# i2Nav-WHU/IC-GVINS

Hardware: AMD Instinct MI355X
Metric: frames/s at 1280x720, 300 feats, 10-KF window; residual/Jacobian eval/s (higher is better)
Workload: dtype u8/int64 front-end (f32/f64 solves), f64 factors

## Files before the change

### ic-gvins_amd/csrc/image.hip

```cpp
#include <algorithm>

#include "icg_internal.h"

#define PRE_MAX_JOBS 64
struct pre_jobs {
    const uint8_t *src[PRE_MAX_JOBS];
    int32_t slot[PRE_MAX_JOBS];
    int stride;
    const int32_t *slot_ind;
};
__device__ __forceinline__ int pre_job_slot(const pre_jobs &j, int b) { return j.slot_ind ? j.slot_ind[b] : j.slot[b]; }

__global__ void k_bgr2gray(const uint8_t *bgr, int w, int h, int sstride, size_t sbatch, uint8_t *gray, int gstride,
                           size_t gbatch) {
    int x = blockIdx.x * blockDim.x + threadIdx.x;
    int y = blockIdx.y;
    int b = blockIdx.z;
    if (x >= w) return;
    const uint8_t *p = bgr + (size_t) b * sbatch + (size_t) y * sstride + 3 * x;
    gray[(size_t) b * gbatch + (size_t) y * gstride + x] =
        (uint8_t) ((p[0] * 1868 + p[1] * 9617 + p[2] * 4899 + 8192) >> 14);
}

__global__ void k_hist256(pre_jobs jobs, int w, int h, unsigned int *hist ) {
    __shared__ unsigned int sh[256];
    int b = blockIdx.y;
    sh[threadIdx.x] = 0;
    __syncthreads();
    const uint8_t *src = jobs.src[b];
    const int stride   = jobs.stride;
    int total          = src ? w * h : 0;
    for (int i = blockIdx.x * blockDim.x + threadIdx.x; i < total; i += gridDim.x * blockDim.x) {
        int y = i / w, x = i - y * w;
        atomicAdd(&sh[src[(size_t) y * stride + x]], 1u);
    }
    __syncthreads();
    if (sh[threadIdx.x]) atomicAdd(&hist[(size_t) b * 256 + threadIdx.x], sh[threadIdx.x]);
}

struct clahe_geom {
    int w, h, tw, th, clip;
    float lut_scale, inv_tw, inv_th;
};

__device__ __forceinline__ int wave_sum_i32(int v) {
    v += __builtin_amdgcn_update_dpp(0, v, 0xB1, 0xF, 0xF, false);
    v += __builtin_amdgcn_update_dpp(0, v, 0x4E, 0xF, 0xF, false);
    v += __builtin_amdgcn_update_dpp(0, v, 0x141, 0xF, 0xF, false);
    v += __builtin_amdgcn_update_dpp(0, v, 0x140, 0xF, 0xF, false);
    v += __builtin_amdgcn_update_dpp(0, v, 0x142, 0xA, 0xF, false);
    v += __builtin_amdgcn_update_dpp(0, v, 0x143, 0xC, 0xF, false);
    return __builtin_amdgcn_readlane(v, 63);
}
__device__ __forceinline__ int wave_scan_i32(int v) {
    v += __builtin_amdgcn_update_dpp(0, v, 0x111, 0xF, 0xF, true);
    v += __builtin_amdgcn_update_dpp(0, v, 0x112, 0xF, 0xF, true);
    v += __builtin_amdgcn_update_dpp(0, v, 0x114, 0xF, 0xF, true);
    v += __builtin_amdgcn_update_dpp(0, v, 0x118, 0xF, 0xF, true);
    v += __builtin_amdgcn_update_dpp(0, v, 0x142, 0xA, 0xF, false);
    v += __builtin_amdgcn_update_dpp(0, v, 0x143, 0xC, 0xF, false);
    return v;
}

__global__ __launch_bounds__(64) void k_clahe_lut(pre_jobs jobs, clahe_geom g, uint8_t *lut , int n_items) {
    __shared__ __attribute__((aligned(16))) unsigned int hist[256];
    const int lane = threadIdx.x;
    const int item = icg_xcd_chunked(blockIdx.x, n_items);
    if (item >= n_items) return;
    const int b    = item / (ICG_CLAHE_TILES * ICG_CLAHE_TILES);
    const int tile = item - b * (ICG_CLAHE_TILES * ICG_CLAHE_TILES);
    const int ty = tile / ICG_CLAHE_TILES, tx = tile - ty * ICG_CLAHE_TILES;
    const uint8_t *src = jobs.src[b];
    if (!src) return;
    const int stride   = jobs.stride;
    reinterpret_cast<uint4 *>(hist)[lane] = make_uint4(0, 0, 0, 0);
    __syncthreads();

    const int x_begin = tx * g.tw, x_end = x_begin + g.tw, y_begin = ty * g.th;
    const int xa  = x_begin & ~3;
    const int ndw = (((x_end + 3) & ~3) - xa) >> 2;
    const bool pad_small = g.th * ICG_CLAHE_TILES < 2 * g.h - 1;
    auto load_row_dword = [&](int r, int x) -> unsigned int {
        const uint8_t *row = src + (size_t) (pad_small ? icg_reflect1(y_begin + r, g.h) : icg_reflect101(y_begin + r, g.h)) * stride;
        if (x + 3 < g.w) return *reinterpret_cast<const unsigned int *>(row + x);
        unsigned int v = 0;
#pragma unroll
        for (int j = 0; j < 4; j++) v |= (unsigned int) row[icg_reflect101(x + j, g.w)] << (8 * j);
        return v;
    };
    const int nin = ndw - 2;
    const bool fast = nin >= 1 && nin <= 16 && y_begin + g.th <= g.h && xa + 4 * ndw <= g.w;
    if (fast) {
        const int d = lane & 15, q = lane >> 4;
        const bool on = d < nin;
        const uint8_t *p = src + (size_t) (y_begin + q) * stride + (xa + 4 * (on ? d + 1 : 1));
        unsigned char *hb = reinterpret_cast<unsigned char *>(hist);
        const size_t step = 4 * (size_t) stride;
        for (int r = q; r < g.th; r += 16, p += 4 * step) {
            unsigned int v[4];
            bool ok[4];
#pragma unroll
            for (int k = 0; k < 4; k++) {
                ok[k] = on && r + 4 * k < g.th;
                v[k]  = r + 4 * k < g.th ? *reinterpret_cast<const unsigned int *>(p + k * step) : 0u;
            }
#pragma unroll
            for (int k = 0; k < 4; k++) {
                if (ok[k]) {
                    atomicAdd(reinterpret_cast<unsigned int *>(hb + ((v[k] << 2) & 0x3fcu)), 1u);
                    atomicAdd(reinterpret_cast<unsigned int *>(hb + ((v[k] >> 6) & 0x3fcu)), 1u);
                    atomicAdd(reinterpret_cast<unsigned int *>(hb + ((v[k] >> 14) & 0x3fcu)), 1u);
                    atomicAdd(reinterpret_cast<unsigned int *>(hb + ((v[k] >> 22) & 0x3fcu)), 1u);
                }
            }
        }
    } else {
        {
            const int items = g.th * (nin > 0 ? nin : 0);
            const unsigned int magic = nin > 0 ? ((1u << 20) + (unsigned int) nin - 1u) / (unsigned int) nin : 0u;
            constexpr int CH = 9;
            for (int base = 0; base < items; base += 64 * CH) {
                unsigned int v[CH];
                bool ok[CH];
    #pragma unroll
                for (int k = 0; k < CH; k++) {
                    const int i = base + k * 64 + lane;
                    ok[k]       = i < items;
                    v[k]        = 0;
                    if (ok[k]) {
                        const int r = (int) (((unsigned int) i * magic) >> 20), d = 1 + i - r * nin;
                        v[k]        = load_row_dword(r, xa + 4 * d);
                    }
                }
    #pragma unroll
                for (int k = 0; k < CH; k++) {
                    if (ok[k]) {
    #pragma unroll
                        for (int j = 0; j < 4; j++) atomicAdd(&hist[(v[k] >> (8 * j)) & 0xff], 1u);
                    }
                }
            }
        }
    }
    {
        const int nedge = ndw >= 2 ? 2 : 1, items = g.th * nedge;
        for (int i = lane; i < items; i += 64) {
            const int r = nedge == 2 ? (i >> 1) : i, d = (nedge == 2 && (i & 1)) ? ndw - 1 : 0;
            const int x = xa + 4 * d;
            const unsigned int v = load_row_dword(r, x);
#pragma unroll
            for (int j = 0; j < 4; j++) {
                const int xx = x + j;
                if (xx >= x_begin && xx < x_end) atomicAdd(&hist[(v >> (8 * j)) & 0xff], 1u);
            }
        }
    }
    __syncthreads();

    const uint4 h4 = reinterpret_cast<const uint4 *>(hist)[lane];
    int hv[4]      = {(int) h4.x, (int) h4.y, (int) h4.z, (int) h4.w};
    int excess     = 0;
#pragma unroll
    for (int j = 0; j < 4; j++) {
        if (hv[j] > g.clip) {
            excess += hv[j] - g.clip;
            hv[j] = g.clip;
        }
    }
    const int clipped   = wave_sum_i32(excess);
    const int batch_add = clipped / 256;
    const int residual  = clipped - batch_add * 256;
    int step            = residual ? 256 / residual : 1;
    if (step < 1) step = 1;
    int run = 0;
#pragma unroll
    for (int j = 0; j < 4; j++) {
        const int t = 4 * lane + j;
        hv[j] += batch_add;
        if (residual != 0 && (t % step) == 0 && (t / step) < residual) hv[j]++;
        run += hv[j];
        hv[j] = run;
    }
    const int incl = wave_scan_i32(run);
    const int excl = incl - run;
    unsigned int packed = 0;
#pragma unroll
    for (int j = 0; j < 4; j++) {
        const float f = rintf((float) (excl + hv[j]) * g.lut_scale);
        int iv        = (int) f;
        iv            = iv < 0 ? 0 : (iv > 255 ? 255 : iv);
        packed |= (unsigned int) iv << (8 * j);
    }
    reinterpret_cast<unsigned int *>(lut + ((size_t) b * ICG_CLAHE_TILES * ICG_CLAHE_TILES + tile) * 256)[lane] = packed;
}

#define CLAHE_CHUNK 256
#define CLAHE_MAXCOLS 24
#define CLAHE_FCOLS 8

typedef float f32x2 __attribute__((ext_vector_type(2)));

template <bool FLT>
__device__ __forceinline__ void clahe_apply_body(const pre_jobs &jobs, const clahe_geom &g, const uint8_t *lut, uint8_t *frames, size_t slot_bytes,
                                                 int dpitch, unsigned int *slut, int strip, int chunk, int b, int t, int dslot, int p_lo, int npairs,
                                                 int x_begin) {
    const int T = ICG_CLAHE_TILES;
    int ty1 = strip - 1, ty2 = strip;
    if (ty1 < 0) ty1 = 0;
    if (ty2 > T - 1) ty2 = T - 1;
    const unsigned int *blut = reinterpret_cast<const unsigned int *>(lut + (size_t) b * T * T * 256);
    for (int i = t; i < npairs * 64; i += 256) {
        const int p = p_lo + (i >> 6), v4 = i & 63;
        int c1 = p - 1, c2 = p;
        if (c1 < 0) c1 = 0;
        if (c2 > T - 1) c2 = T - 1;
        const unsigned int A = blut[(ty1 * T + c1) * 64 + v4], B = blut[(ty1 * T + c2) * 64 + v4];
        const unsigned int C = blut[(ty2 * T + c1) * 64 + v4], D = blut[(ty2 * T + c2) * 64 + v4];
        if (FLT) {
            float4 *dst = reinterpret_cast<float4 *>(slut) + 4 * i;
#define CL_F(w, k) ((float) (((w) >> (8 * (k))) & 0xffu))
            dst[0] = make_float4(CL_F(A, 0), CL_F(B, 0), CL_F(C, 0), CL_F(D, 0));
            dst[1] = make_float4(CL_F(A, 1), CL_F(B, 1), CL_F(C, 1), CL_F(D, 1));
            dst[2] = make_float4(CL_F(A, 2), CL_F(B, 2), CL_F(C, 2), CL_F(D, 2));
            dst[3] = make_float4(CL_F(A, 3), CL_F(B, 3), CL_F(C, 3), CL_F(D, 3));
#undef CL_F
        } else {
            const unsigned int ab01 = __builtin_amdgcn_perm(B, A, 0x05010400u), ab23 = __builtin_amdgcn_perm(B, A, 0x07030602u);
            const unsigned int cd01 = __builtin_amdgcn_perm(D, C, 0x05010400u), cd23 = __builtin_amdgcn_perm(D, C, 0x07030602u);
            uint4 e;
            e.x = __builtin_amdgcn_perm(cd01, ab01, 0x05040100u);
            e.y = __builtin_amdgcn_perm(cd01, ab01, 0x07060302u);
            e.z = __builtin_amdgcn_perm(cd23, ab23, 0x05040100u);
            e.w = __builtin_amdgcn_perm(cd23, ab23, 0x07060302u);
            reinterpret_cast<uint4 *>(slut)[i] = e;
        }
    }
    __syncthreads();

    const int wave = t >> 6, lane = t & 63;
    const int x0 = x_begin + lane * 4;
    int pofs[4];
    float xa[4], xa1[4];
#pragma unroll
    for (int k = 0; k < 4; k++) {
        const int x     = x0 + k;
        const float txf = x * g.inv_tw - 0.5f;
        const int tx1   = (int) floorf(txf);
        xa[k]           = txf - tx1;
        xa1[k]          = 1.0f - xa[k];
        int p           = tx1 + 1 - p_lo;
        p               = p < 0 ? 0 : (p > npairs - 1 ? npairs - 1 : p);
        pofs[k]         = p << 8;
    }
    if (x0 >= g.w) return;

    int y_lo = (strip - 1) * g.th + g.th / 2 - 2;
    int y_hi = strip * g.th + g.th / 2 + 3;
    if (y_lo < 0) y_lo = 0;
    if (y_hi > g.h) y_hi = g.h;
    const uint8_t *src = jobs.src[b];
    const int stride   = jobs.stride;
    uint8_t *dst       = frames + (size_t) dslot * slot_bytes;
    if (FLT) {
        const float4 *sf = reinterpret_cast<const float4 *>(slut);
        for (int y = y_lo + wave; y < y_hi; y += 4) {
            const float tyf = y * g.inv_th - 0.5f;
            const int tyr   = (int) floorf(tyf);
            if (tyr != strip - 1) continue;
            const float ya = tyf - tyr, ya1 = 1.0f - ya;
            const unsigned int pin = *reinterpret_cast<const unsigned int *>(src + (size_t) y * stride + x0);
            const float4 e0 = sf[pofs[0] + (pin & 0xff)], e1 = sf[pofs[1] + ((pin >> 8) & 0xff)];
            const float4 e2 = sf[pofs[2] + ((pin >> 16) & 0xff)], e3 = sf[pofs[3] + (pin >> 24)];
            const float r0 = (e0.x * xa1[0] + e0.y * xa[0]) * ya1 + (e0.z * xa1[0] + e0.w * xa[0]) * ya;
            const float r1 = (e1.x * xa1[1] + e1.y * xa[1]) * ya1 + (e1.z * xa1[1] + e1.w * xa[1]) * ya;
            const float r2 = (e2.x * xa1[2] + e2.y * xa[2]) * ya1 + (e2.z * xa1[2] + e2.w * xa[2]) * ya;
            const float r3 = (e3.x * xa1[3] + e3.y * xa[3]) * ya1 + (e3.z * xa1[3] + e3.w * xa[3]) * ya;
            const unsigned int m0 = __float_as_uint(r0 + 12582912.f), m1 = __float_as_uint(r1 + 12582912.f);
            const unsigned int m2 = __float_as_uint(r2 + 12582912.f), m3 = __float_as_uint(r3 + 12582912.f);
            const unsigned int lo = __builtin_amdgcn_perm(m1, m0, 0x0c0c0400u), hi = __builtin_amdgcn_perm(m3, m2, 0x0c0c0400u);
            *reinterpret_cast<unsigned int *>(dst + (size_t) y * dpitch + x0) = __builtin_amdgcn_perm(hi, lo, 0x05040100u);
        }
        return;
    }
    const f32x2 XA01 = {xa[0], xa[1]}, XA23 = {xa[2], xa[3]}, XB01 = {xa1[0], xa1[1]}, XB23 = {xa1[2], xa1[3]};
    for (int y = y_lo + wave; y < y_hi; y += 4) {
        const float tyf = y * g.inv_th - 0.5f;
        const int tyr   = (int) floorf(tyf);
        if (tyr != strip - 1) continue;
        const float ya = tyf - tyr, ya1 = 1.0f - ya;
        const unsigned int pin = *reinterpret_cast<const unsigned int *>(src + (size_t) y * stride + x0);
        const unsigned int e0 = slut[pofs[0] + (pin & 0xff)], e1 = slut[pofs[1] + ((pin >> 8) & 0xff)];
        const unsigned int e2 = slut[pofs[2] + ((pin >> 16) & 0xff)], e3 = slut[pofs[3] + (pin >> 24)];
#define CL_B(e, k) ((float) (((e) >> (8 * (k))) & 0xffu))
        const f32x2 A01 = {CL_B(e0, 0), CL_B(e1, 0)}, B01 = {CL_B(e0, 1), CL_B(e1, 1)};
        const f32x2 C01 = {CL_B(e0, 2), CL_B(e1, 2)}, D01 = {CL_B(e0, 3), CL_B(e1, 3)};
        const f32x2 A23 = {CL_B(e2, 0), CL_B(e3, 0)}, B23 = {CL_B(e2, 1), CL_B(e3, 1)};
        const f32x2 C23 = {CL_B(e2, 2), CL_B(e3, 2)}, D23 = {CL_B(e2, 3), CL_B(e3, 3)};
#undef CL_B
        const f32x2 r01 = (A01 * XB01 + B01 * XA01) * ya1 + (C01 * XB01 + D01 * XA01) * ya;
        const f32x2 r23 = (A23 * XB23 + B23 * XA23) * ya1 + (C23 * XB23 + D23 * XA23) * ya;
        const float res[4] = {r01.x, r01.y, r23.x, r23.y};
        unsigned int pout = 0;
#pragma unroll
        for (int k = 0; k < 4; k++) {
            const int iv = (int) rintf(res[k]);
            pout |= (unsigned int) (iv < 0 ? 0 : (iv > 255 ? 255 : iv)) << (8 * k);
        }
        *reinterpret_cast<unsigned int *>(dst + (size_t) y * dpitch + x0) = pout;
    }
}

__global__ __launch_bounds__(256) void k_clahe_apply(pre_jobs jobs, clahe_geom g, const uint8_t *lut, uint8_t *frames,
                                                     size_t slot_bytes, int dpitch) {
    __shared__ __attribute__((aligned(16))) unsigned int slut[CLAHE_FCOLS * 256 * 4];
    static_assert(CLAHE_FCOLS * 4 >= CLAHE_MAXCOLS, "the byte form must fit the same array");
    const int strip = blockIdx.x;
    const int chunk = blockIdx.y;
    const int b     = blockIdx.z;
    const int t     = threadIdx.x;
    const int dslot = pre_job_slot(jobs, b);
    if (!jobs.src[b] || dslot < 0) return;
    const int x_begin = chunk * CLAHE_CHUNK;
    int x_end         = x_begin + CLAHE_CHUNK;
    if (x_end > g.w) x_end = g.w;
    const int p_lo   = (int) floorf(x_begin * g.inv_tw - 0.5f) + 1;
    const int p_hi   = (int) floorf((x_end - 1) * g.inv_tw - 0.5f) + 1;
    const int npairs = p_hi - p_lo + 1;
    if (npairs <= CLAHE_FCOLS)
        clahe_apply_body<true>(jobs, g, lut, frames, slot_bytes, dpitch, slut, strip, chunk, b, t, dslot, p_lo, npairs, x_begin);
    else
        clahe_apply_body<false>(jobs, g, lut, frames, slot_bytes, dpitch, slut, strip, chunk, b, t, dslot, p_lo, npairs, x_begin);
}

#define PR_STRIP_OUT 128
struct pr_sel {
    unsigned int a, b, t, v;
};
typedef unsigned int pr_u3 __attribute__((ext_vector_type(3)));
__device__ __forceinline__ pr_u3 pr_load(const uint8_t *row, unsigned int wx) {
    typedef pr_u3 __attribute__((aligned(4))) u3a;
    return *reinterpret_cast<const u3a *>(row + wx);
}
template <bool EDGE> __device__ __forceinline__ unsigned int pr_hsum(const pr_u3 E, const pr_sel &S) {
    unsigned int A, B, V4;
    if (EDGE) {
        A  = __builtin_amdgcn_perm(E.y, E.x, S.a);
        B  = __builtin_amdgcn_perm(E.y, E.x, S.b);
        V4 = __builtin_amdgcn_perm(E.z, __builtin_amdgcn_perm(E.y, E.x, S.t), S.v);
    } else {
        A  = __builtin_amdgcn_alignbyte(E.y, E.x, 2);
        B  = E.y;
        V4 = E.z & 0xffu;
    }
    const unsigned int h0 = __builtin_amdgcn_udot4(B, 0x00010000u, __builtin_amdgcn_udot4(A, 0x04060401u, 0u, false), false);
    const unsigned int h1 = __builtin_amdgcn_udot4(B, 0x04060401u, V4, false);
    return h0 | (h1 << 16);
}

template <bool EDGE>
__device__ __forceinline__ void pr_band(const uint8_t *src, int sh, int spitch, uint8_t *dst, int dpitch, int i0, int i1, unsigned int wx,
                                        const pr_sel &S, unsigned int dcol, bool store) {
    auto srow = [&](int r) { return src + (unsigned int) __builtin_amdgcn_readfirstlane(icg_reflect1(r, sh) * spitch); };
    unsigned int hA = pr_hsum<EDGE>(pr_load(srow(2 * i0 - 2), wx), S), hB = pr_hsum<EDGE>(pr_load(srow(2 * i0 - 1), wx), S);
    unsigned int hC = pr_hsum<EDGE>(pr_load(srow(2 * i0), wx), S);
    pr_u3 R1 = pr_load(srow(2 * i0 + 1), wx), R2 = pr_load(srow(2 * i0 + 2), wx);
    for (int i = i0; i < i1; i++) {
        const pr_u3 N1 = pr_load(srow(2 * i + 3), wx), N2 = pr_load(srow(2 * i + 4), wx);
        const unsigned int hD = pr_hsum<EDGE>(R1, S), hE = pr_hsum<EDGE>(R2, S);
        unsigned int v = hA + hE;
        v              = ((hB + hD) << 2) + v;
        v += (hC << 2) + (hC + hC);
        v += 0x00800080u;
        if (store) *reinterpret_cast<unsigned short *>(dst + (size_t) i * dpitch + dcol) = (unsigned short) __builtin_amdgcn_perm(v, v, 0x0c0c0301u);
        hA = hC, hB = hD, hC = hE;
        R1 = N1, R2 = N2;
    }
}

__global__ __launch_bounds__(64) void k_pyrdown_rows(uint8_t *frames, size_t slot_bytes, pre_jobs jobs, unsigned int src_off, int sw, int sh,
                                                     int spitch, unsigned int dst_off, int dw, int dh, int dpitch, int n_strips, int n_bands,
                                                     int band_rows, int n_tasks) {
    const int task = icg_xcd_chunked(blockIdx.x, n_tasks);
    if (task >= n_tasks) return;
    const int per_job = n_strips * n_bands;
    const int job = task / per_job, rem = task - job * per_job;
    const int band = rem / n_strips, strip = rem - band * n_strips;
    const int dslot = __builtin_amdgcn_readfirstlane(pre_job_slot(jobs, job));
    if (dslot < 0) return;
    uint8_t *slot = frames + (size_t) dslot * slot_bytes;
    const int lane = threadIdx.x;
    const int oj   = strip * PR_STRIP_OUT + 2 * lane;
    const int x  = min(2 * oj, (sw - 1) & ~3);
    const int wx = max(x - 4, 0);
    const bool edge = strip == 0 || 2 * (strip + 1) * PR_STRIP_OUT + 4 > sw;
    pr_sel S;
    S.a = S.b = S.t = S.v = 0;
    if (edge) {
        int ix[7];
#pragma unroll
        for (int k = 0; k < 7; k++) ix[k] = min(max(icg_reflect101(x - 2 + k, sw) - wx, 0), 11);
        S.a = (unsigned int) (ix[0] & 7) | ((unsigned int) (ix[1] & 7) << 8) | ((unsigned int) (ix[2] & 7) << 16) | ((unsigned int) (ix[3] & 7) << 24);
        S.b = (unsigned int) (ix[2] & 7) | ((unsigned int) (ix[3] & 7) << 8) | ((unsigned int) (ix[4] & 7) << 16) | ((unsigned int) (ix[5] & 7) << 24);
        S.t = 0x0c0c0c00u | (unsigned int) (ix[6] & 7);
        S.v = ix[6] >= 8 ? (0x0c0c0c04u + (unsigned int) (ix[6] - 8)) : 0x0c0c0c00u;
    }
    const int i0 = band * band_rows, i1 = min(i0 + band_rows, dh);
    if (i0 >= i1) return;
    const uint8_t *src = slot + src_off;
    uint8_t *dst       = slot + dst_off;
    const bool store   = oj < dw;
    if (edge)
        pr_band<true>(src, sh, spitch, dst, dpitch, i0, i1, (unsigned int) wx, S, (unsigned int) oj, store);
    else
        pr_band<false>(src, sh, spitch, dst, dpitch, i0, i1, (unsigned int) wx, S, (unsigned int) oj, store);
}

__global__ void k_hist_mean(int n, const unsigned int *hist, int w, int h, double *mean) {
    const int k = blockIdx.x * blockDim.x + threadIdx.x;
    if (k >= n) return;
    double acc = 0;
    for (int i = 0; i < 256; i++) {
        const float hf = (float) hist[(size_t) k * 256 + i];
        acc += hf * (float) i / 256.0;
    }
    mean[k] = acc / ((double) w * h);
}

static int preprocess_impl(icg_ctx *ctx, int n, const int32_t *slots, const int32_t *d_slot_ind, const uint8_t *const *images, int stride, int channels,
                           int src_on_device, double *hist_mean, double *d_hist_mean) {
    if (!ctx || n < 0 || (n > 0 && ((!slots && !d_slot_ind) || !images))) return ICG_ERR_INVALID;
    if (n == 0) return ICG_OK;
    if (n > ctx->cfg.max_batch) return icg_fail(ctx, ICG_ERR_CAPACITY, "preprocess batch %d > max_batch %d", n, ctx->cfg.max_batch);
    if (channels != 1 && channels != 3) return icg_fail(ctx, ICG_ERR_INVALID, "channels must be 1 or 3");
    const int w = ctx->cfg.width, h = ctx->cfg.height;
    if (stride < w * channels) return icg_fail(ctx, ICG_ERR_INVALID, "stride too small");
    for (int k = 0; k < n && slots; k++)
        if (slots[k] < 0 || slots[k] >= ctx->cfg.n_slots || !images[k]) return icg_fail(ctx, ICG_ERR_INVALID, "bad slot/image %d", k);
    ICG_HIP(ctx, hipSetDevice(ctx->cfg.device));
    const bool want_hist = hist_mean || d_hist_mean;

    const int T = ICG_CLAHE_TILES;
    int ew = w, eh = h;
    if (w % T != 0 || h % T != 0) {
        ew = w + (T - w % T);
        eh = h + (T - h % T);
    }
    clahe_geom g;
    g.w = w;
    g.h = h;
    g.tw = ew / T;
    g.th = eh / T;
    int area    = g.tw * g.th;
    g.lut_scale = 255.0f / area;
    g.clip      = (int) (3.0 * area / 256);
    if (g.clip < 1) g.clip = 1;
    g.inv_tw = 1.0f / g.tw;
    g.inv_th = 1.0f / g.th;
    if (CLAHE_CHUNK / g.tw + 3 > CLAHE_MAXCOLS)
        return icg_fail(ctx, ICG_ERR_INVALID, "image too small for CLAHE chunking (tile width %d)", g.tw);

    const size_t raw_batch = (size_t) ctx->raw_pitch * h;
    hipMemcpyKind kind     = src_on_device ? hipMemcpyDeviceToDevice : hipMemcpyHostToDevice;
    unsigned int *d_hist   = nullptr;
    if (want_hist) {
        if (int rcd = icg_arena_drain(ctx)) return rcd;
        ctx->arena_off = 0;
        int rc         = icg_arena_reserve(ctx, sizeof(unsigned int) * 256 * (size_t) n + 4096);
        if (rc) return rc;
        d_hist = icg_d<unsigned int>(ctx, icg_arena_alloc(ctx, sizeof(unsigned int) * 256 * (size_t) n));
        if ((rc = icg_arena_overflow_check(ctx))) return rc;
        ICG_HIP(ctx, hipMemsetAsync(d_hist, 0, sizeof(unsigned int) * 256 * (size_t) n, ctx->stream));
    }

    for (int base = 0; base < n; base += PRE_MAX_JOBS) {
        const int m = std::min(PRE_MAX_JOBS, n - base);
        pre_jobs jobs;
        memset(&jobs, 0, sizeof jobs);
        for (int k = 0; k < m && slots; k++) jobs.slot[k] = slots[base + k];
        jobs.slot_ind = d_slot_ind ? d_slot_ind + base : nullptr;
        if (channels == 3) {
            if (!ctx->d_bgr) ICG_HIP(ctx, hipMalloc((void **) &ctx->d_bgr, (size_t) w * 3 * h * ctx->cfg.max_batch));
            for (int k = 0; k < m; k++)
                if (images[base + k])
                    ICG_HIP(ctx, hipMemcpy2DAsync(ctx->d_bgr + (size_t) (base + k) * w * 3 * h, (size_t) w * 3, images[base + k], stride,
                                                  (size_t) w * 3, h, kind, ctx->stream));
            icg_prof_scope ps(ctx, "bgr2gray");
            hipLaunchKernelGGL(k_bgr2gray, dim3((w + 255) / 256, h, m), dim3(256), 0, ctx->stream,
                               ctx->d_bgr + (size_t) base * w * 3 * h, w, h, w * 3, (size_t) w * 3 * h,
                               ctx->d_raw + (size_t) base * raw_batch, ctx->raw_pitch, raw_batch);
            for (int k = 0; k < m; k++) jobs.src[k] = images[base + k] ? ctx->d_raw + (size_t) (base + k) * raw_batch : nullptr;
            jobs.stride = ctx->raw_pitch;
        } else {
            bool direct = src_on_device && (stride % 4 == 0);
            for (int k = 0; k < m && direct; k++) direct = (((uintptr_t) images[base + k]) % 4) == 0;
            if (direct) {
                for (int k = 0; k < m; k++) jobs.src[k] = images[base + k];
                jobs.stride = stride;
            } else {
                const bool linear = stride == w && ctx->raw_pitch == w;
                for (int k = 0; k < m; k++) {
                    uint8_t *dst = ctx->d_raw + (size_t) (base + k) * raw_batch;
                    if (!images[base + k]) {
                        jobs.src[k] = nullptr;
                        continue;
                    }
                    if (linear)
                        ICG_HIP(ctx, hipMemcpyAsync(dst, images[base + k], (size_t) w * h, kind, ctx->stream));
                    else
                        ICG_HIP(ctx, hipMemcpy2DAsync(dst, ctx->raw_pitch, images[base + k], stride, w, h, kind, ctx->stream));
                    jobs.src[k] = dst;
                }
                jobs.stride = ctx->raw_pitch;
            }
        }
        if (want_hist) {
            icg_prof_scope ps(ctx, "hist256");
            hipLaunchKernelGGL(k_hist256, dim3(64, m), dim3(256), 0, ctx->stream, jobs, w, h, d_hist + (size_t) base * 256);
        }
        uint8_t *lut = ctx->d_lut + (size_t) base * T * T * 256;
        {
            icg_prof_scope ps(ctx, "clahe_lut");
            hipLaunchKernelGGL(k_clahe_lut, dim3(icg_xcd_grid(T * T * m)), dim3(64), 0, ctx->stream, jobs, g, lut, T * T * m);
        }
        {
            icg_prof_scope ps(ctx, "clahe_apply");
            hipLaunchKernelGGL(k_clahe_apply, dim3(T + 1, (w + CLAHE_CHUNK - 1) / CLAHE_CHUNK, m), dim3(256), 0, ctx->stream, jobs,
                               g, lut, ctx->d_frames, ctx->slot_bytes, ctx->lv[0].pitch);
        }
        for (int l = 1; l < ctx->n_levels; l++) {
            icg_prof_scope ps(ctx, "pyrdown_rows");
            const icg_level &a = ctx->lv[l - 1], &bb = ctx->lv[l];
            const int n_strips = (bb.w + PR_STRIP_OUT - 1) / PR_STRIP_OUT;
            const int band_rows = bb.h >= 256 ? 32 : bb.h >= 128 ? 16 : 8;
            const int n_bands   = (bb.h + band_rows - 1) / band_rows;
            const int n_tasks   = n_strips * n_bands * m;
            hipLaunchKernelGGL(k_pyrdown_rows, dim3(icg_xcd_grid(n_tasks)), dim3(64), 0, ctx->stream, ctx->d_frames, ctx->slot_bytes, jobs,
                               (unsigned int) a.off, a.w, a.h, a.pitch, (unsigned int) bb.off, bb.w, bb.h, bb.pitch, n_strips, n_bands, band_rows,
                               n_tasks);
        }
    }
    if (d_hist_mean) hipLaunchKernelGGL(k_hist_mean, dim3((n + 63) / 64), dim3(64), 0, ctx->stream, n, d_hist, w, h, d_hist_mean);
    ICG_HIP(ctx, hipGetLastError());
    if (d_hist_mean) ctx->arena_off = 0;
    if (!hist_mean) return ICG_OK;

    std::vector<unsigned int> hc((size_t) n * 256);
    ICG_HIP(ctx, hipMemcpyAsync(hc.data(), d_hist, sizeof(unsigned int) * 256 * (size_t) n, hipMemcpyDeviceToHost, ctx->stream));
    ICG_HIP(ctx, hipStreamSynchronize(ctx->stream));
    icg_prof_collect(ctx);
    for (int k = 0; k < n; k++) {
        double acc = 0;
        for (int i = 0; i < 256; i++) {
            float hf = (float) hc[(size_t) k * 256 + i];
            acc += hf * (float) i / 256.0;
        }
        hist_mean[k] = acc / ((double) w * h);
    }
    ctx->arena_off = 0;
    return ICG_OK;
}

extern "C" int icg_frames_preprocess(icg_ctx *ctx, int n, const int32_t *slots, const uint8_t *const *images, int stride, int channels,
                                     int src_on_device, double *hist_mean) {
    if (n > 0 && !slots) return ICG_ERR_INVALID;
    return preprocess_impl(ctx, n, slots, nullptr, images, stride, channels, src_on_device, hist_mean, nullptr);
}

int icg_preprocess_launch_ind(icg_ctx *ctx, int n, const int32_t *d_slot_ind, const uint8_t *const *images, int stride, int channels,
                              int src_on_device, double *d_hist_mean) {
    return preprocess_impl(ctx, n, nullptr, d_slot_ind, images, stride, channels, src_on_device, nullptr, d_hist_mean);
}

extern "C" int icg_frame_download(icg_ctx *ctx, int slot, int level, uint8_t *dst, int dst_stride) {
    if (!ctx || !dst || slot < 0 || slot >= ctx->cfg.n_slots || level < 0 || level >= ctx->n_levels) return ICG_ERR_INVALID;
    ICG_HIP(ctx, hipSetDevice(ctx->cfg.device));
    const icg_level &L = ctx->lv[level];
    if (dst_stride < L.w) return ICG_ERR_INVALID;
    ICG_HIP(ctx, hipStreamSynchronize(ctx->stream));
    ICG_HIP(ctx, hipMemcpy2D(dst, dst_stride, ctx->d_frames + (size_t) slot * ctx->slot_bytes + L.off, L.pitch, L.w, L.h,
                             hipMemcpyDeviceToHost));
    return ICG_OK;
}
```

Before: 159,200.

## Compute CLAHE LUTs per tile-row with multi-wave blocks and full-width coalesced loads

The CLAHE histogram kernel now assigns one block of four waves to a whole row of tiles instead of one single-wave block per tile. Each lane reads full-width dword columns and bins pixels into per-tile shared histograms, using magic-number division to find the tile for each column. Edge columns are handled in a separate pass. The job batch size is also raised from 64 to 256, so more images go into each launch. The aim is coalesced row reads, fewer blocks, and no per-tile edge handling, at the cost of more shared memory per block and reliance on the reflect1 padding path for every case.

Result: no change. 159,600, median of 6 (+0.3%).

```diff
diff --git a/ic-gvins_amd/csrc/image.hip b/ic-gvins_amd/csrc/image.hip
--- a/ic-gvins_amd/csrc/image.hip
+++ b/ic-gvins_amd/csrc/image.hip
@@ -2,7 +2,7 @@
 
 #include "icg_internal.h"
 
-#define PRE_MAX_JOBS 64
+#define PRE_MAX_JOBS 256
 struct pre_jobs {
     const uint8_t *src[PRE_MAX_JOBS];
     int32_t slot[PRE_MAX_JOBS];
@@ -41,6 +41,7 @@
 struct clahe_geom {
     int w, h, tw, th, clip;
     float lut_scale, inv_tw, inv_th;
+    unsigned int tw_magic;
 };
 
 __device__ __forceinline__ int wave_sum_i32(int v) {
@@ -62,136 +63,97 @@
     return v;
 }
 
-__global__ __launch_bounds__(64) void k_clahe_lut(pre_jobs jobs, clahe_geom g, uint8_t *lut , int n_items) {
-    __shared__ __attribute__((aligned(16))) unsigned int hist[256];
-    const int lane = threadIdx.x;
+#define CLAHE_LUT_WAVES 4
+#define CLAHE_LUT_ROWS 4
+__global__ __launch_bounds__(64 * CLAHE_LUT_WAVES) void k_clahe_lut(pre_jobs jobs, clahe_geom g, uint8_t *lut , int n_items) {
+    constexpr int T = ICG_CLAHE_TILES, NW = CLAHE_LUT_WAVES, U = CLAHE_LUT_ROWS;
+    __shared__ __attribute__((aligned(16))) unsigned int hist[T * 256];
+    const int lane = threadIdx.x & 63, wave = __builtin_amdgcn_readfirstlane(threadIdx.x >> 6);
     const int item = icg_xcd_chunked(blockIdx.x, n_items);
     if (item >= n_items) return;
-    const int b    = item / (ICG_CLAHE_TILES * ICG_CLAHE_TILES);
-    const int tile = item - b * (ICG_CLAHE_TILES * ICG_CLAHE_TILES);
-    const int ty = tile / ICG_CLAHE_TILES, tx = tile - ty * ICG_CLAHE_TILES;
+    const int b = item / T, ty = item - b * T;
     const uint8_t *src = jobs.src[b];
     if (!src) return;
-    const int stride   = jobs.stride;
-    reinterpret_cast<uint4 *>(hist)[lane] = make_uint4(0, 0, 0, 0);
+    const int stride = jobs.stride;
+    for (int i = threadIdx.x; i < T * 64; i += 64 * NW) reinterpret_cast<uint4 *>(hist)[i] = make_uint4(0, 0, 0, 0);
     __syncthreads();
 
-    const int x_begin = tx * g.tw, x_end = x_begin + g.tw, y_begin = ty * g.th;
-    const int xa  = x_begin & ~3;
-    const int ndw = (((x_end + 3) & ~3) - xa) >> 2;
-    const bool pad_small = g.th * ICG_CLAHE_TILES < 2 * g.h - 1;
-    auto load_row_dword = [&](int r, int x) -> unsigned int {
-        const uint8_t *row = src + (size_t) (pad_small ? icg_reflect1(y_begin + r, g.h) : icg_reflect101(y_begin + r, g.h)) * stride;
-        if (x + 3 < g.w) return *reinterpret_cast<const unsigned int *>(row + x);
-        unsigned int v = 0;
-#pragma unroll
-        for (int j = 0; j < 4; j++) v |= (unsigned int) row[icg_reflect101(x + j, g.w)] << (8 * j);
-        return v;
-    };
-    const int nin = ndw - 2;
-    const bool fast = nin >= 1 && nin <= 16 && y_begin + g.th <= g.h && xa + 4 * ndw <= g.w;
-    if (fast) {
-        const int d = lane & 15, q = lane >> 4;
-        const bool on = d < nin;
-        const uint8_t *p = src + (size_t) (y_begin + q) * stride + (xa + 4 * (on ? d + 1 : 1));
-        unsigned char *hb = reinterpret_cast<unsigned char *>(hist);
-        const size_t step = 4 * (size_t) stride;
-        for (int r = q; r < g.th; r += 16, p += 4 * step) {
-            unsigned int v[4];
-            bool ok[4];
-#pragma unroll
-            for (int k = 0; k < 4; k++) {
-                ok[k] = on && r + 4 * k < g.th;
-                v[k]  = r + 4 * k < g.th ? *reinterpret_cast<const unsigned int *>(p + k * step) : 0u;
-            }
-#pragma unroll
-            for (int k = 0; k < 4; k++) {
-                if (ok[k]) {
-                    atomicAdd(reinterpret_cast<unsigned int *>(hb + ((v[k] << 2) & 0x3fcu)), 1u);
-                    atomicAdd(reinterpret_cast<unsigned int *>(hb + ((v[k] >> 6) & 0x3fcu)), 1u);
-                    atomicAdd(reinterpret_cast<unsigned int *>(hb + ((v[k] >> 14) & 0x3fcu)), 1u);
-                    atomicAdd(reinterpret_cast<unsigned int *>(hb + ((v[k] >> 22) & 0x3fcu)), 1u);
-                }
-            }
-        }
-    } else {
-        {
-            const int items = g.th * (nin > 0 ? nin : 0);
-            const unsigned int magic = nin > 0 ? ((1u << 20) + (unsigned int) nin - 1u) / (unsigned int) nin : 0u;
-            constexpr int CH = 9;
-            for (int base = 0; base < items; base += 64 * CH) {
-                unsigned int v[CH];
-                bool ok[CH];
-    #pragma unroll
-                for (int k = 0; k < CH; k++) {
-                    const int i = base + k * 64 + lane;
-                    ok[k]       = i < items;
-                    v[k]        = 0;
-                    if (ok[k]) {
-                        const int r = (int) (((unsigned int) i * magic) >> 20), d = 1 + i - r * nin;
-                        v[k]        = load_row_dword(r, xa + 4 * d);
-                    }
-                }
-    #pragma unroll
-                for (int k = 0; k < CH; k++) {
-                    if (ok[k]) {
-    #pragma unroll
-                        for (int j = 0; j < 4; j++) atomicAdd(&hist[(v[k] >> (8 * j)) & 0xff], 1u);
+    unsigned char *hb = reinterpret_cast<unsigned char *>(hist);
+    const int y_begin = ty * g.th;
+    auto srow = [&](int r) { return src + (unsigned int) __builtin_amdgcn_readfirstlane(icg_reflect1(y_begin + r, g.h) * stride); };
+    const int ndwf = g.w >> 2;
+    for (int c0 = 0; c0 < ndwf; c0 += 64) {
+        const int c = c0 + lane;
+        if (c < ndwf) {
+            const unsigned int x = 4u * c;
+            const int tx0 = icg_div_by_magic((int) x, g.tw_magic);
+            const int nb  = (tx0 + 1) * g.tw - (int) x;
+            const unsigned int b0 = (unsigned int) tx0 << 10, b1 = (unsigned int) (tx0 + (nb <= 1)) << 10;
+            const unsigned int b2 = (unsigned int) (tx0 + (nb <= 2)) << 10, b3 = (unsigned int) (tx0 + (nb <= 3)) << 10;
+            for (int r = wave; r < g.th; r += U * NW) {
+                unsigned int v[U];
+#pragma unroll
+                for (int k = 0; k < U; k++) v[k] = r + k * NW < g.th ? *reinterpret_cast<const unsigned int *>(srow(r + k * NW) + x) : 0u;
+#pragma unroll
+                for (int k = 0; k < U; k++) {
+                    if (r + k * NW < g.th) {
+                        atomicAdd(reinterpret_cast<unsigned int *>(hb + b0 + (__builtin_amdgcn_perm(0u, v[k], 0x0c0c0c00u) << 2)), 1u);
+                        atomicAdd(reinterpret_cast<unsigned int *>(hb + b1 + (((v[k] >> 8) & 0xffu) << 2)), 1u);
+                        atomicAdd(reinterpret_cast<unsigned int *>(hb + b2 + (((v[k] >> 16) & 0xffu) << 2)), 1u);
+                        atomicAdd(reinterpret_cast<unsigned int *>(hb + b3 + ((v[k] >> 24) << 2)), 1u);
                     }
                 }
             }
         }
     }
-    {
-        const int nedge = ndw >= 2 ? 2 : 1, items = g.th * nedge;
-        for (int i = lane; i < items; i += 64) {
-            const int r = nedge == 2 ? (i >> 1) : i, d = (nedge == 2 && (i & 1)) ? ndw - 1 : 0;
-            const int x = xa + 4 * d;
-            const unsigned int v = load_row_dword(r, x);
-#pragma unroll
-            for (int j = 0; j < 4; j++) {
-                const int xx = x + j;
-                if (xx >= x_begin && xx < x_end) atomicAdd(&hist[(v >> (8 * j)) & 0xff], 1u);
-            }
+    const int x_edge = 4 * ndwf, n_edge = g.tw * T - x_edge;
+    if ((lane & 31) < n_edge) {
+        const int x = x_edge + (lane & 31);
+        const uint8_t *col = src + icg_reflect1(x, g.w);
+        const unsigned int be = (unsigned int) icg_div_by_magic(x, g.tw_magic) << 10;
+        for (int r = 2 * wave + (lane >> 5); r < g.th; r += 2 * NW) {
+            atomicAdd(reinterpret_cast<unsigned int *>(hb + be + 4u * col[(size_t) icg_reflect1(y_begin + r, g.h) * stride]), 1u);
         }
     }
     __syncthreads();
 
-    const uint4 h4 = reinterpret_cast<const uint4 *>(hist)[lane];
-    int hv[4]      = {(int) h4.x, (int) h4.y, (int) h4.z, (int) h4.w};
-    int excess     = 0;
-#pragma unroll
-    for (int j = 0; j < 4; j++) {
-        if (hv[j] > g.clip) {
-            excess += hv[j] - g.clip;
-            hv[j] = g.clip;
-        }
-    }
-    const int clipped   = wave_sum_i32(excess);
-    const int batch_add = clipped / 256;
-    const int residual  = clipped - batch_add * 256;
-    int step            = residual ? 256 / residual : 1;
-    if (step < 1) step = 1;
-    int run = 0;
-#pragma unroll
-    for (int j = 0; j < 4; j++) {
-        const int t = 4 * lane + j;
-        hv[j] += batch_add;
-        if (residual != 0 && (t % step) == 0 && (t / step) < residual) hv[j]++;
-        run += hv[j];
-        hv[j] = run;
-    }
-    const int incl = wave_scan_i32(run);
-    const int excl = incl - run;
-    unsigned int packed = 0;
-#pragma unroll
-    for (int j = 0; j < 4; j++) {
-        const float f = rintf((float) (excl + hv[j]) * g.lut_scale);
-        int iv        = (int) f;
-        iv            = iv < 0 ? 0 : (iv > 255 ? 255 : iv);
-        packed |= (unsigned int) iv << (8 * j);
-    }
-    reinterpret_cast<unsigned int *>(lut + ((size_t) b * ICG_CLAHE_TILES * ICG_CLAHE_TILES + tile) * 256)[lane] = packed;
+    for (int tx = wave; tx < T; tx += NW) {
+        const uint4 h4 = reinterpret_cast<const uint4 *>(hist)[tx * 64 + lane];
+        int hv[4]      = {(int) h4.x, (int) h4.y, (int) h4.z, (int) h4.w};
+        int excess     = 0;
+#pragma unroll
+        for (int j = 0; j < 4; j++) {
+            excess += max(hv[j] - g.clip, 0);
+            hv[j] = min(hv[j], g.clip);
+        }
+        const int clipped   = wave_sum_i32(excess);
+        const int batch_add = clipped / 256;
+        const int residual  = clipped - batch_add * 256;
+        int step            = residual ? 256 / residual : 1;
+        if (step < 1) step = 1;
+        const unsigned int step_magic = 65535u / (unsigned int) step + 1u;
+        int run = 0;
+#pragma unroll
+        for (int j = 0; j < 4; j++) {
+            const unsigned int t = 4u * lane + j;
+            const unsigned int q = __umul24(t, step_magic) >> 16;
+            hv[j] += batch_add;
+            if (residual != 0 && __umul24(q, (unsigned int) step) == t && (int) q < residual) hv[j]++;
+            run += hv[j];
+            hv[j] = run;
+        }
+        const int incl = wave_scan_i32(run);
+        const int excl = incl - run;
+        unsigned int packed = 0;
+#pragma unroll
+        for (int j = 0; j < 4; j++) {
+            const float f = rintf((float) (excl + hv[j]) * g.lut_scale);
+            int iv        = (int) f;
+            iv            = iv < 0 ? 0 : (iv > 255 ? 255 : iv);
+            packed |= (unsigned int) iv << (8 * j);
+        }
+        reinterpret_cast<unsigned int *>(lut + ((size_t) b * T * T + ty * T + tx) * 256)[lane] = packed;
+    }
 }
 
 #define CLAHE_CHUNK 256
@@ -456,6 +418,7 @@
     if (g.clip < 1) g.clip = 1;
     g.inv_tw = 1.0f / g.tw;
     g.inv_th = 1.0f / g.th;
+    g.tw_magic = icg_div_magic(g.tw);
     if (CLAHE_CHUNK / g.tw + 3 > CLAHE_MAXCOLS)
         return icg_fail(ctx, ICG_ERR_INVALID, "image too small for CLAHE chunking (tile width %d)", g.tw);
 
@@ -520,7 +483,7 @@
         uint8_t *lut = ctx->d_lut + (size_t) base * T * T * 256;
         {
             icg_prof_scope ps(ctx, "clahe_lut");
-            hipLaunchKernelGGL(k_clahe_lut, dim3(icg_xcd_grid(T * T * m)), dim3(64), 0, ctx->stream, jobs, g, lut, T * T * m);
+            hipLaunchKernelGGL(k_clahe_lut, dim3(icg_xcd_grid(T * m)), dim3(64 * CLAHE_LUT_WAVES), 0, ctx->stream, jobs, g, lut, T * m);
         }
         {
             icg_prof_scope ps(ctx, "clahe_apply");
```
